# Lightning-AI/lit-llama

Hardware: NVIDIA H100
Metric: LLaMA-7B gptq.int4 decode tokens/sec (higher is better)
Workload: dtype bf16

## Files before the change

lit-llama_b200/csrc/attention.cu:

```cuda
#include <cstdlib>

#include "b2l_common.cuh"

namespace b2l {

__global__ void ring_advance_kernel(const int64_t* __restrict__ input_pos, int T, int32_t* ring_start, int S) {
  if (threadIdx.x == 0 && blockIdx.x == 0) {
    if (input_pos[T - 1] >= (int64_t)S) *ring_start = (*ring_start + 1) % S;
  }
}

__global__ void rope_append_kernel(__nv_bfloat16* __restrict__ qkv, __nv_bfloat16* __restrict__ k_cache,
                                   __nv_bfloat16* __restrict__ v_cache, const float* __restrict__ rope,
                                   const int64_t* __restrict__ input_pos, const int32_t* __restrict__ ring_start,
                                   int T, int n_head, int hs, int S, int block_size, int rope_rows) {
  const int bt = blockIdx.x, h = blockIdx.y, b = bt / T, t = bt % T;
  const int C = n_head * hs;
  long long p = input_pos ? input_pos[t] : (long long)t;
  const long long prow = rope_rows ? (long long)t : (p < block_size ? p : (long long)block_size - 1);
  __nv_bfloat16* q = qkv + (size_t)bt * 3 * C + h * hs;
  __nv_bfloat16* k = q + C;
  const __nv_bfloat16* v = q + 2 * C;
  __nv_bfloat16 *kd = k, *vd = nullptr;
  if (k_cache != nullptr) {
    const int w = (int)(p < S ? p : (long long)S - 1);
    const int phys = (w + *ring_start) % S;
    const size_t off = (((size_t)b * n_head + h) * S + phys) * hs;
    kd = k_cache + off;
    vd = v_cache + off;
  }
  for (int i = threadIdx.x; i < hs / 2; i += blockDim.x) {
    const float c = rope[((size_t)prow * (hs / 2) + i) * 2 + 0];
    const float s = rope[((size_t)prow * (hs / 2) + i) * 2 + 1];
    const float q0 = bf2f(q[2 * i]), q1 = bf2f(q[2 * i + 1]);
    const float k0 = bf2f(k[2 * i]), k1 = bf2f(k[2 * i + 1]);
    q[2 * i] = f2bf(__fsub_rn(__fmul_rn(q0, c), __fmul_rn(q1, s)));
    q[2 * i + 1] = f2bf(__fadd_rn(__fmul_rn(q1, c), __fmul_rn(q0, s)));
    kd[2 * i] = f2bf(__fsub_rn(__fmul_rn(k0, c), __fmul_rn(k1, s)));
    kd[2 * i + 1] = f2bf(__fadd_rn(__fmul_rn(k1, c), __fmul_rn(k0, s)));
    if (vd != nullptr) {
      vd[2 * i] = v[2 * i];
      vd[2 * i + 1] = v[2 * i + 1];
    }
  }
}

struct KvView {
  const __nv_bfloat16* k;
  const __nv_bfloat16* v;
  size_t b_stride, h_stride, s_stride;
  int S;
};

constexpr int ATT_WARPS = 4;
constexpr int ATT_MAX_EPL = 8;

template <int EPL>
__global__ void __launch_bounds__(ATT_WARPS * 32)
    attn_partial_kernel(const __nv_bfloat16* __restrict__ qkv, KvView kv, const int64_t* __restrict__ input_pos,
                        const int32_t* __restrict__ ring_start, float* __restrict__ work, int T, int n_head,
                        int hs, int n_split, int chunk) {
  const int bh = blockIdx.x, b = bh / n_head, h = bh % n_head, t = blockIdx.y, sp = blockIdx.z;
  const int lane = threadIdx.x & 31, warp = threadIdx.x >> 5;
  const int C = n_head * hs;
  long long p = input_pos ? input_pos[t] : (long long)t;
  const int cap = kv.S > 0 ? kv.S : T;
  const int L = (int)(p < cap ? p : (long long)cap - 1) + 1;
  const int ring = (kv.S > 0 && ring_start) ? *ring_start : 0;
  const int j0 = sp * chunk, j1 = min(L, j0 + chunk);
  float* out = work + (((size_t)bh * T + t) * n_split + sp) * (hs + 2);
  if (j0 >= j1) {
    if (threadIdx.x == 0) { out[0] = -INFINITY; out[1] = 0.f; }
    for (int d = threadIdx.x; d < hs; d += blockDim.x) out[2 + d] = 0.f;
    return;
  }
  const float scale = rsqrtf((float)hs);
  float qv[ATT_MAX_EPL];
  const __nv_bfloat16* q = qkv + ((size_t)b * T + t) * 3 * C + h * hs;
#pragma unroll
  for (int e = 0; e < ATT_MAX_EPL; ++e) {
    int d = (EPL > 0) ? lane * EPL + e : lane + 32 * e;
    qv[e] = (e < (EPL > 0 ? EPL : ATT_MAX_EPL) && d < hs) ? bf2f(q[d]) * scale : 0.f;
// ... 16 lines not shown
      kx[2] = __uint_as_float(ku.y << 16); kx[3] = __uint_as_float(ku.y & 0xffff0000u);
      vx[0] = __uint_as_float(vu.x << 16); vx[1] = __uint_as_float(vu.x & 0xffff0000u);
      vx[2] = __uint_as_float(vu.y << 16); vx[3] = __uint_as_float(vu.y & 0xffff0000u);
    } else {
#pragma unroll
      for (int e = 0; e < ATT_MAX_EPL; ++e) {
        int d = lane + 32 * e;
        kx[e] = d < hs ? bf2f(kr[d]) : 0.f;
        vx[e] = d < hs ? bf2f(vr[d]) : 0.f;
      }
    }
    float sc = 0.f;
#pragma unroll
    for (int e = 0; e < (EPL > 0 ? EPL : ATT_MAX_EPL); ++e) sc = fmaf(qv[e], kx[e], sc);
    sc = warp_sum(sc);
    const float mn = fmaxf(m, sc);
    const float corr = __expf(m - mn), pj = __expf(sc - mn);
    l = l * corr + pj;
#pragma unroll
    for (int e = 0; e < (EPL > 0 ? EPL : ATT_MAX_EPL); ++e) acc[e] = fmaf(pj, vx[e], acc[e] * corr);
    m = mn;
  }
  __shared__ float sm_m[ATT_WARPS], sm_l[ATT_WARPS];
  __shared__ float sm_acc[ATT_WARPS][32 * ATT_MAX_EPL];
  if (lane == 0) { sm_m[warp] = m; sm_l[warp] = l; }
#pragma unroll
  for (int e = 0; e < (EPL > 0 ? EPL : ATT_MAX_EPL); ++e) {
    int d = (EPL > 0) ? lane * EPL + e : lane + 32 * e;
    sm_acc[warp][d] = acc[e];
  }
  __syncthreads();
  float M = -INFINITY;
#pragma unroll
  for (int w = 0; w < ATT_WARPS; ++w) M = fmaxf(M, sm_m[w]);
  float Ls = 0.f;
  float wgt[ATT_WARPS];
#pragma unroll
  for (int w = 0; w < ATT_WARPS; ++w) {
    wgt[w] = (sm_m[w] == -INFINITY) ? 0.f : __expf(sm_m[w] - M);
    Ls += sm_l[w] * wgt[w];
  }
  if (threadIdx.x == 0) { out[0] = M; out[1] = Ls; }
  for (int d = threadIdx.x; d < hs; d += blockDim.x) {
    float a = 0.f;
#pragma unroll
    for (int w = 0; w < ATT_WARPS; ++w) a += sm_acc[w][d] * wgt[w];
    out[2 + d] = a;
  }
}

__global__ void attn_combine_kernel(const float* __restrict__ work, __nv_bfloat16* __restrict__ y, int T,
                                    int n_head, int hs, int n_split) {
  pdl_launch_dependents();
  const int bh = blockIdx.x, b = bh / n_head, h = bh % n_head, t = blockIdx.y;
  const float* base = work + ((size_t)bh * T + t) * n_split * (hs + 2);
  float M = -INFINITY;
  for (int s = 0; s < n_split; ++s) M = fmaxf(M, base[(size_t)s * (hs + 2)]);
  float Ls = 0.f;
  for (int s = 0; s < n_split; ++s) {
    float ms = base[(size_t)s * (hs + 2)];
    if (ms != -INFINITY) Ls += base[(size_t)s * (hs + 2) + 1] * __expf(ms - M);
  }
  const float inv = 1.0f / Ls;
  __nv_bfloat16* yr = y + ((size_t)b * T + t) * (n_head * hs) + h * hs;
  for (int d = threadIdx.x; d < hs; d += blockDim.x) {
    float a = 0.f;
    for (int s = 0; s < n_split; ++s) {
      float ms = base[(size_t)s * (hs + 2)];
      if (ms != -INFINITY) a += base[(size_t)s * (hs + 2) + 2 + d] * __expf(ms - M);
    }
    yr[d] = f2bf(a * inv);
  }
}

__global__ void kv_unroll_kernel(const __nv_bfloat16* __restrict__ cache, const int32_t* __restrict__ ring_start,
                                 __nv_bfloat16* __restrict__ out, int S, int hs) {
  const int ring = *ring_start;
  const int phys = (blockIdx.y + ring) % S;
  const __nv_bfloat16* src = cache + ((size_t)blockIdx.x * S + phys) * hs;
  __nv_bfloat16* dst = out + ((size_t)blockIdx.x * S + blockIdx.y) * hs;
  for (int d = threadIdx.x; d < hs; d += blockDim.x) dst[d] = src[d];
}

constexpr int FD_CHUNK = 256;
constexpr int FD_SUB = 64;
constexpr int FD_WARPS = 8;
constexpr int FD_CTAS_PER_SM = 3;
constexpr int WS_CHUNK = FD_SUB;

__device__ __forceinline__ void bf16x8_to_f32(const uint4& u, float* f) {
  const uint32_t w[4] = {u.x, u.y, u.z, u.w};
#pragma unroll
  for (int i = 0; i < 4; ++i) {
    f[2 * i] = __uint_as_float(w[i] << 16);
    f[2 * i + 1] = __uint_as_float(w[i] & 0xffff0000u);
  }
}

__device__ __forceinline__ uint32_t fd_smem_u32(const void* p) { return (uint32_t)__cvta_generic_to_shared(p); }
__device__ __forceinline__ void fd_bulk(uint32_t dst, const void* src, uint32_t bytes, uint32_t bar) {
  asm volatile("cp.async.bulk.shared::cluster.global.mbarrier::complete_tx::bytes [%0], [%1], %2, [%3];" ::"r"(dst), "l"(src), "r"(bytes), "r"(bar) : "memory");
}

constexpr int FD_SUB_BYTES = FD_SUB * 128 * 2;
constexpr int FD_SMEM_BYTES = 4 * FD_SUB_BYTES + FD_WARPS * 128 * 4 + 2 * FD_WARPS * 4 + 16;

__device__ __forceinline__ float fd_adapter_prefix(const float* sq, float* ssc, const __nv_bfloat16* __restrict__ ak,
                                                   const __nv_bfloat16* __restrict__ av, int alen, int warp, int lane,
                                                   int d, bool writer) {
  constexpr int HS = 128;
  const float4 qv = reinterpret_cast<const float4*>(sq)[lane];
#pragma unroll 2
  for (int j = warp; j < alen; j += FD_WARPS) {
    const uint2 ku = __ldg(reinterpret_cast<const uint2*>(ak + (size_t)j * HS) + lane);
    float s = qv.x * __uint_as_float(ku.x << 16);
    s = fmaf(qv.y, __uint_as_float(ku.x & 0xffff0000u), s);
    s = fmaf(qv.z, __uint_as_float(ku.y << 16), s);
    s = fmaf(qv.w, __uint_as_float(ku.y & 0xffff0000u), s);
    s = warp_sum(s);
    if (lane == 0) ssc[j] = s;
  }
  __syncthreads();
  float ay = 0.f;
  if (writer) {
    float mx = -INFINITY;
    for (int j = 0; j < alen; ++j) mx = fmaxf(mx, ssc[j]);
    float l = 0.f;
#pragma unroll 8
    for (int j = 0; j < alen; ++j) {
      const float p = __expf(ssc[j] - mx);
      l += p;
      ay = fmaf(p, bf2f(av[(size_t)j * HS + d]), ay);
    }
    ay /= l;
  }
  return ay;
}

__device__ __forceinline__ __nv_bfloat16 adapter_combine(float y, float ay, float gate) {
  return f2bf(rbf(y) + rbf(gate * rbf(ay)));
}

template <bool ADAPTER>
__global__ void __launch_bounds__(FD_WARPS * 32, ADAPTER ? FD_CTAS_PER_SM : 0)
    attn_decode_fused_kernel(const __nv_bfloat16* qkv, __nv_bfloat16* __restrict__ k_cache,
                             __nv_bfloat16* __restrict__ v_cache, const float* __restrict__ rope,
                             const int64_t* __restrict__ input_pos, const int32_t* __restrict__ ring_start,
                             __nv_bfloat16* __restrict__ y, float* __restrict__ work, int* __restrict__ tickets,
                             int n_head, int S, int block_size, int n_split, unsigned long long* tl, int pre_tiles,
                             int smem_merge, int target_ctas, const __nv_bfloat16* __restrict__ pre_k,
                             const __nv_bfloat16* __restrict__ pre_v, const __nv_bfloat16* __restrict__ pre_gate,
                             int pre_len) {
  constexpr int HS = 128;
  extern __shared__ __align__(128) uint8_t fsm[];
  float* sm_acc = reinterpret_cast<float*>(fsm + 4 * FD_SUB_BYTES);
  float* sm_m = sm_acc + FD_WARPS * HS;
  float* sm_l = sm_m + FD_WARPS;
  unsigned long long* bars = reinterpret_cast<unsigned long long*>(sm_l + FD_WARPS);
  __shared__ int sm_last;

  if (threadIdx.x == 0) tl_min(tl, 0);
  const int bh = blockIdx.x, b = bh / n_head, h = bh % n_head, sp = blockIdx.y;
  unsigned long long* tl0 = (tl != nullptr && blockIdx.x == 0 && blockIdx.y == 0 && threadIdx.x == 0) ? tl + 8 : nullptr;
  int tli = 0;
  auto stamp = [&]() { if (tl0 != nullptr && tli < 24) tl0[tli++] = globaltimer_ns(); };
  stamp();
  const int lane = threadIdx.x & 31, warp = threadIdx.x >> 5;
  const int C = n_head * HS;
  const size_t head_base = ((size_t)b * n_head + h) * S * HS;

  const long long p = input_pos[0];
  const int w_slot = (int)(p < S ? p : (long long)S - 1);
  const int L = w_slot + 1;
  const int want_splits = max(1, target_ctas / n_head);
  const int chunk = L <= FD_CHUNK ? FD_CHUNK
                                  : min(FD_CHUNK, max(FD_SUB, FD_SUB * ((L + FD_SUB * want_splits - 1) / (FD_SUB * want_splits))));
  const int n_active = (L + chunk - 1) / chunk;
  if (sp >= n_active) return;
  const int ring = *ring_start;
  const int j0 = sp * chunk, j1 = min(L, j0 + chunk);
  const int n_old = min(j1, L - 1) - j0;
  const int n_sub = (n_old + FD_SUB - 1) / FD_SUB;
  const bool has_new = (w_slot >= j0 && w_slot < j1);

  const uint32_t bar0 = fd_smem_u32(bars);
  auto request = [&](int i) {
    const int buf = i & 1;
    const int cnt = min(FD_SUB, n_old - i * FD_SUB);
    int phys0 = j0 + i * FD_SUB + ring; if (phys0 >= S) phys0 -= S;
    const int first = min(cnt, S - phys0);
    const uint32_t bar = bar0 + buf * 8;
    const uint32_t kd = fd_smem_u32(fsm) + buf * 2 * FD_SUB_BYTES, vd = kd + FD_SUB_BYTES;
    asm volatile("mbarrier.arrive.expect_tx.shared::cta.b64 _, [%0], %1;" ::"r"(bar), "r"((uint32_t)cnt * HS * 2 * 2) : "memory");
    fd_bulk(kd, k_cache + head_base + (size_t)phys0 * HS, (uint32_t)first * HS * 2, bar);
    fd_bulk(vd, v_cache + head_base + (size_t)phys0 * HS, (uint32_t)first * HS * 2, bar);
    if (first < cnt) {
      fd_bulk(kd + first * HS * 2, k_cache + head_base, (uint32_t)(cnt - first) * HS * 2, bar);
      fd_bulk(vd + first * HS * 2, v_cache + head_base, (uint32_t)(cnt - first) * HS * 2, bar);
    }
  };
  const int pre = (n_active == 1) ? 2 : pre_tiles;
  if (threadIdx.x == 0) {
    asm volatile("mbarrier.init.shared::cta.b64 [%0], 1;" ::"r"(bar0) : "memory");
    asm volatile("mbarrier.init.shared::cta.b64 [%0], 1;" ::"r"(bar0 + 8) : "memory");
    asm volatile("fence.mbarrier_init.release.cluster;" ::: "memory");
    if (n_sub > 0) request(0);
    if (pre > 1 && n_sub > 1) request(1);
  }
  if constexpr (ADAPTER) {
    if (threadIdx.x == 0) {
      const size_t off = (size_t)h * pre_len * HS;
      const uint32_t bytes = (uint32_t)pre_len * HS * 2;
      asm volatile("cp.async.bulk.prefetch.L2.global [%0], %1;" ::"l"(pre_k + off), "r"(bytes) : "memory");
      asm volatile("cp.async.bulk.prefetch.L2.global [%0], %1;" ::"l"(pre_v + off), "r"(bytes) : "memory");
    }
  }
  const long long prow = p < block_size ? p : (long long)block_size - 1;
  const int grp = lane >> 3, sub = lane & 7, d0 = sub * 16;
  float cs[16];
  {
    const float4* rp = reinterpret_cast<const float4*>(rope + ((size_t)prow * (HS / 2) + d0 / 2) * 2);
#pragma unroll
    for (int i = 0; i < 4; ++i) {
      float4 t = rp[i];
      cs[4 * i] = t.x; cs[4 * i + 1] = t.y; cs[4 * i + 2] = t.z; cs[4 * i + 3] = t.w;
    }
  }
  __syncthreads();
  pdl_wait();
  if (threadIdx.x == 0) tl_max(tl, 1);
  stamp();
  pdl_launch_dependents();

  const __nv_bfloat16* qrow = qkv + (size_t)b * 3 * C + h * HS + d0;
  float q[16];
  {
    float raw[16];
    const uint4 qa = ld_coherent_u4(qrow), qb = ld_coherent_u4(qrow + 8);
    if (threadIdx.x == 0 && pre <= 1 && n_sub > 1) request(1);
    bf16x8_to_f32(qa, raw);
    bf16x8_to_f32(qb, raw + 8);
    const float scale = rsqrtf((float)HS);
#pragma unroll
    for (int i = 0; i < 8; ++i) {
      const float c = cs[2 * i], s_ = cs[2 * i + 1];
      const float e = rbf(__fsub_rn(__fmul_rn(raw[2 * i], c), __fmul_rn(raw[2 * i + 1], s_)));
      const float o = rbf(__fadd_rn(__fmul_rn(raw[2 * i + 1], c), __fmul_rn(raw[2 * i], s_)));
      q[2 * i] = e * scale;
      q[2 * i + 1] = o * scale;
    }
  }
  float ay = 0.f;
  if constexpr (ADAPTER) {
    if (warp == 0 && grp == 0) {
      float4* dq = reinterpret_cast<float4*>(sm_acc + d0);
#pragma unroll
      for (int i = 0; i < 4; ++i) dq[i] = make_float4(q[4 * i], q[4 * i + 1], q[4 * i + 2], q[4 * i + 3]);
    }
    __syncthreads();
    ay = fd_adapter_prefix(sm_acc, sm_acc + HS, pre_k + (size_t)h * pre_len * HS, pre_v + (size_t)h * pre_len * HS,
                           pre_len, warp, lane, threadIdx.x & (HS - 1), threadIdx.x < HS);
  }

  float m = -INFINITY, l = 0.f, acc[16];
#pragma unroll
  for (int i = 0; i < 16; ++i) acc[i] = 0.f;
  if (tl0 != nullptr && q[0] != 12345.678f) stamp();
  if (has_new && warp == 0 && grp == 0) {
    int phys = w_slot + ring; if (phys >= S) phys -= S;
    float raw[16], kf[16], vf[16];
    bf16x8_to_f32(ld_coherent_u4(qrow + C), raw);
    bf16x8_to_f32(ld_coherent_u4(qrow + C + 8), raw + 8);
    uint32_t out[8];
#pragma unroll
    for (int i = 0; i < 8; ++i) {
      const float c = cs[2 * i], s_ = cs[2 * i + 1];
      kf[2 * i] = rbf(__fsub_rn(__fmul_rn(raw[2 * i], c), __fmul_rn(raw[2 * i + 1], s_)));
      kf[2 * i + 1] = rbf(__fadd_rn(__fmul_rn(raw[2 * i + 1], c), __fmul_rn(raw[2 * i], s_)));
      out[i] = (__float_as_uint(kf[2 * i]) >> 16) | (__float_as_uint(kf[2 * i + 1]) & 0xffff0000u);
    }
    const uint4 va = ld_coherent_u4(qrow + 2 * C), vb = ld_coherent_u4(qrow + 2 * C + 8);
    uint4* kd = reinterpret_cast<uint4*>(k_cache + head_base + (size_t)phys * HS + d0);
    uint4* vd = reinterpret_cast<uint4*>(v_cache + head_base + (size_t)phys * HS + d0);
    kd[0] = make_uint4(out[0], out[1], out[2], out[3]); kd[1] = make_uint4(out[4], out[5], out[6], out[7]);
    vd[0] = va; vd[1] = vb;
    bf16x8_to_f32(va, vf); bf16x8_to_f32(vb, vf + 8);
    float sc = 0.f;
#pragma unroll
    for (int e = 0; e < 16; ++e) sc = fmaf(q[e], kf[e], sc);
    sc += __shfl_xor_sync(0x000000ffu, sc, 1);
    sc += __shfl_xor_sync(0x000000ffu, sc, 2);
    sc += __shfl_xor_sync(0x000000ffu, sc, 4);
    const float mn = fmaxf(m, sc);
    const float corr = __expf(m - mn), pj = __expf(sc - mn);
    l = l * corr + pj;
#pragma unroll
    for (int e = 0; e < 16; ++e) acc[e] = fmaf(pj, vf[e], acc[e] * corr);
    m = mn;
  }
  for (int i = 0; i < n_sub; ++i) {
    const int buf = i & 1;
    const int cnt = min(FD_SUB, n_old - i * FD_SUB);
    {
      uint32_t ok;
      const uint32_t par = (uint32_t)(i >> 1) & 1u;
      do {
        asm volatile("{\n\t.reg .pred p;\n\tmbarrier.try_wait.parity.shared::cta.b64 p, [%1], %2;\n\tselp.u32 %0, 1, 0, p;\n\t}" : "=r"(ok) : "r"(bar0 + buf * 8), "r"(par) : "memory");
      } while (!ok);
    }
    const __nv_bfloat16* kt = reinterpret_cast<const __nv_bfloat16*>(fsm + buf * 2 * FD_SUB_BYTES);
    const __nv_bfloat16* vt = kt + FD_SUB * HS;
    stamp();
    float sc[2];
    bool valid[2];
    const uint4* vr[2];
#pragma unroll
    for (int it = 0; it < 2; ++it) {
      const int r = warp * 8 + it * 4 + grp;
      valid[it] = r < cnt;
      const int rc = valid[it] ? r : 0;
      const uint4* kr = reinterpret_cast<const uint4*>(kt + (size_t)rc * HS + d0);
      vr[it] = reinterpret_cast<const uint4*>(vt + (size_t)rc * HS + d0);
      float kf[16];
      bf16x8_to_f32(kr[0], kf); bf16x8_to_f32(kr[1], kf + 8);
      float a0 = 0.f, a1 = 0.f;
#pragma unroll
      for (int e = 0; e < 8; ++e) { a0 = fmaf(q[e], kf[e], a0); a1 = fmaf(q[8 + e], kf[8 + e], a1); }
      sc[it] = a0 + a1;
    }
#pragma unroll
    for (int o = 1; o <= 4; o <<= 1) {
      sc[0] += __shfl_xor_sync(0xffffffffu, sc[0], o);
      sc[1] += __shfl_xor_sync(0xffffffffu, sc[1], o);
    }
    {
      const float s0 = valid[0] ? sc[0] : -INFINITY, s1 = valid[1] ? sc[1] : -INFINITY;
      const float mn = fmaxf(m, fmaxf(s0, s1));
      if (mn != -INFINITY) {
        const float corr = __expf(m - mn), p0 = __expf(s0 - mn), p1 = __expf(s1 - mn);
        float v0[16], v1[16];
        bf16x8_to_f32(vr[0][0], v0); bf16x8_to_f32(vr[0][1], v0 + 8);
        bf16x8_to_f32(vr[1][0], v1); bf16x8_to_f32(vr[1][1], v1 + 8);
        l = l * corr + p0 + p1;
#pragma unroll
        for (int e = 0; e < 16; ++e) acc[e] = fmaf(p1, v1[e], fmaf(p0, v0[e], acc[e] * corr));
        m = mn;
      }
    }
    __syncthreads();
    stamp();
    if (threadIdx.x == 0 && i + 2 < n_sub) request(i + 2);
  }
  if (threadIdx.x == 0) tl_max(tl, 2);
  __syncwarp();
  if (threadIdx.x == 0) tl_max(tl, 3);
  float* part = reinterpret_cast<float*>(fsm);
  float* pm = part + 32 * HS;
  float* pl = pm + 32, *pw = pl + 32;
  const int n_part = smem_merge ? 32 : FD_WARPS;
  if (smem_merge) {
    const int g = warp * 4 + grp;
    float4* dst = reinterpret_cast<float4*>(part + g * HS + d0);
#pragma unroll
    for (int i = 0; i < 4; ++i) dst[i] = make_float4(acc[4 * i], acc[4 * i + 1], acc[4 * i + 2], acc[4 * i + 3]);
    if (sub == 0) { pm[g] = m; pl[g] = l; }
  } else {
#pragma unroll
    for (int off = 8; off <= 16; off <<= 1) {
      const float mo = __shfl_xor_sync(0xffffffffu, m, off);
      const float lo = __shfl_xor_sync(0xffffffffu, l, off);
      const float mn = fmaxf(m, mo);
      const float ca = (m == -INFINITY) ? 0.f : __expf(m - mn);
      const float cb = (mo == -INFINITY) ? 0.f : __expf(mo - mn);
      l = l * ca + lo * cb;
#pragma unroll
      for (int i = 0; i < 16; ++i) {
        const float ao = __shfl_xor_sync(0xffffffffu, acc[i], off);
        acc[i] = acc[i] * ca + ao * cb;
      }
      m = mn;
    }
    if (lane == 0) { pm[warp] = m; pl[warp] = l; }
    if (grp == 0) {
      float4* dst = reinterpret_cast<float4*>(part + warp * HS + d0);
#pragma unroll
      for (int i = 0; i < 4; ++i) dst[i] = make_float4(acc[4 * i], acc[4 * i + 1], acc[4 * i + 2], acc[4 * i + 3]);
    }
  }
  __syncthreads();
  if (warp == 0) {
    const float mi = lane < n_part ? pm[lane] : -INFINITY;
    const float Mx = warp_max(mi);
    const float wi = (mi == -INFINITY) ? 0.f : __expf(mi - Mx);
    const float Lx = warp_sum(lane < n_part ? pl[lane] * wi : 0.f);
    pw[lane] = wi;
    if (lane == 0) { pw[32] = Mx; pw[33] = Lx; }
  }
  __syncthreads();
  const float M = pw[32], Ls = pw[33];
  const int d = threadIdx.x & (HS - 1);
  const bool writer = threadIdx.x < HS;
  float a = 0.f;
  if (writer) {
#pragma unroll 8
    for (int g = 0; g < n_part; ++g) a = fmaf(part[g * HS + d], pw[g], a);
  }
  stamp();
  if (n_active == 1) {
    if constexpr (ADAPTER) {
      if (writer) y[(size_t)b * C + h * HS + d] = adapter_combine(a / Ls, ay, bf2f(pre_gate[h]));
    } else {
      if (writer) y[(size_t)b * C + h * HS + d] = f2bf(a / Ls);
    }
    if (threadIdx.x == 0) tl_max(tl, 4);
    stamp();
    return;
  }
  float* out = work + ((size_t)bh * n_split + sp) * (HS + 2);
  if (threadIdx.x == 0) { out[0] = M; out[1] = Ls; }
  if (writer) out[2 + d] = a;
  __syncthreads();
  if (threadIdx.x == 0) {
    int t;
    asm volatile("atom.add.acq_rel.gpu.global.s32 %0, [%1], 1;" : "=r"(t) : "l"(tickets + bh) : "memory");
    sm_last = (t == n_active - 1);
    if (sm_last) tickets[bh] = 0;
  }
  __syncthreads();
  stamp();
  if (!sm_last) return;
  const float* base = work + (size_t)bh * n_split * (HS + 2);
  float MM = -INFINITY, LL = 0.f, aa = 0.f;
  for (int s0 = 0; s0 < n_active; s0 += 8) {
    float ms[8], ls[8], as[8];
#pragma unroll
    for (int i = 0; i < 8; ++i) {
      const int s2 = s0 + i;
      const bool ok = s2 < n_active;
      const float* bp = base + (size_t)(ok ? s2 : s0) * (HS + 2);
      ms[i] = ok ? __ldcg(bp) : -INFINITY;
      ls[i] = ok ? __ldcg(bp + 1) : 0.f;
      as[i] = ok ? __ldcg(bp + 2 + d) : 0.f;
    }
    float bm = MM;
#pragma unroll
    for (int i = 0; i < 8; ++i) bm = fmaxf(bm, ms[i]);
    const float c0 = (MM == -INFINITY) ? 0.f : __expf(MM - bm);
    LL *= c0; aa *= c0;
#pragma unroll
    for (int i = 0; i < 8; ++i) {
      const float wg = (ms[i] == -INFINITY) ? 0.f : __expf(ms[i] - bm);
      LL += ls[i] * wg;
      aa += as[i] * wg;
    }
    MM = bm;
  }
  if constexpr (ADAPTER) {
    if (writer) y[(size_t)b * C + h * HS + d] = adapter_combine(aa / LL, ay, bf2f(pre_gate[h]));
  } else {
    if (writer) y[(size_t)b * C + h * HS + d] = f2bf(aa / LL);
  }
  if (threadIdx.x == 0) tl_max(tl, 4);
}

__global__ void __launch_bounds__(ATT_WARPS * 32)
    attn_adapter_prefix_kernel(const __nv_bfloat16* __restrict__ qkv, const __nv_bfloat16* __restrict__ pk,
                               const __nv_bfloat16* __restrict__ pv, const __nv_bfloat16* __restrict__ gate,
                               __nv_bfloat16* __restrict__ y, int n_head, int hs, int alen) {
  pdl_launch_dependents();
  __shared__ float sq[32 * ATT_MAX_EPL];
  __shared__ float ssc[B2L_ADAPTER_MAX_LEN];
  const int bt = blockIdx.x, h = blockIdx.y;
  const int lane = threadIdx.x & 31, warp = threadIdx.x >> 5;
  const int C = n_head * hs;
  const float scale = rsqrtf((float)hs);
  const __nv_bfloat16* q = qkv + (size_t)bt * 3 * C + h * hs;
  for (int d = threadIdx.x; d < hs; d += blockDim.x) sq[d] = bf2f(q[d]) * scale;
  __syncthreads();
  const __nv_bfloat16* kb = pk + (size_t)h * alen * hs;
  const __nv_bfloat16* vb = pv + (size_t)h * alen * hs;
  for (int j = warp; j < alen; j += ATT_WARPS) {
    float s = 0.f;
    for (int d = lane; d < hs; d += 32) s = fmaf(sq[d], bf2f(kb[(size_t)j * hs + d]), s);
    s = warp_sum(s);
    if (lane == 0) ssc[j] = s;
  }
  __syncthreads();
  float mx = -INFINITY;
  for (int j = 0; j < alen; ++j) mx = fmaxf(mx, ssc[j]);
  float l = 0.f;
  for (int j = 0; j < alen; ++j) l += __expf(ssc[j] - mx);
  const float g = bf2f(gate[h]);
  __nv_bfloat16* yr = y + (size_t)bt * C + h * hs;
  for (int d = threadIdx.x; d < hs; d += blockDim.x) {
    float a = 0.f;
    for (int j = 0; j < alen; ++j) a = fmaf(__expf(ssc[j] - mx), bf2f(vb[(size_t)j * hs + d]), a);
    yr[d] = adapter_combine(bf2f(yr[d]), a / l, g);
  }
}

constexpr int PF_Q = 64, PF_K = 64, PF_LD = 136;
constexpr int PF_TILE_BYTES = PF_Q * PF_LD * 2;
constexpr int PF_SMEM_BYTES = 5 * PF_TILE_BYTES;

__device__ __forceinline__ void ldsm_x4(uint32_t addr, uint32_t& r0, uint32_t& r1, uint32_t& r2, uint32_t& r3) {
  asm volatile("ldmatrix.sync.aligned.m8n8.x4.shared.b16 {%0, %1, %2, %3}, [%4];" : "=r"(r0), "=r"(r1), "=r"(r2), "=r"(r3) : "r"(addr) : "memory");
}
__device__ __forceinline__ void ldsm_x4_t(uint32_t addr, uint32_t& r0, uint32_t& r1, uint32_t& r2, uint32_t& r3) {
  asm volatile("ldmatrix.sync.aligned.m8n8.x4.trans.shared.b16 {%0, %1, %2, %3}, [%4];" : "=r"(r0), "=r"(r1), "=r"(r2), "=r"(r3) : "r"(addr) : "memory");
}
__device__ __forceinline__ void mma_bf16(float (&d)[4], uint32_t a0, uint32_t a1, uint32_t a2, uint32_t a3, uint32_t b0, uint32_t b1) {
  asm volatile("mma.sync.aligned.m16n8k16.row.col.f32.bf16.bf16.f32 {%0, %1, %2, %3}, {%4, %5, %6, %7}, {%8, %9}, {%0, %1, %2, %3};"
               : "+f"(d[0]), "+f"(d[1]), "+f"(d[2]), "+f"(d[3]) : "r"(a0), "r"(a1), "r"(a2), "r"(a3), "r"(b0), "r"(b1));
}
__device__ __forceinline__ void pf_cp16(uint32_t dst, const void* src) {
  asm volatile("cp.async.cg.shared.global [%0], [%1], 16;" ::"r"(dst), "l"(src) : "memory");
}
__device__ __forceinline__ void split_bf16x2(float x, float y, uint32_t& hi, uint32_t& lo) {
  const __nv_bfloat162 h = __floats2bfloat162_rn(x, y);
  const __nv_bfloat162 l = __floats2bfloat162_rn(x - __low2float(h), y - __high2float(h));
  hi = *reinterpret_cast<const uint32_t*>(&h);
  lo = *reinterpret_cast<const uint32_t*>(&l);
}

__global__ void __launch_bounds__(128)
    attn_prefill_kernel(const __nv_bfloat16* __restrict__ qkv, KvView kv, const int64_t* __restrict__ input_pos,
                        const int32_t* __restrict__ ring_start, __nv_bfloat16* __restrict__ y, int T, int n_head) {
  constexpr int HS = 128;
  extern __shared__ __align__(128) uint8_t psm[];
  const uint32_t sq = fd_smem_u32(psm), sk0 = sq + PF_TILE_BYTES;
  const int bh = blockIdx.x, b = bh / n_head, h = bh % n_head, t0 = blockIdx.y * PF_Q;
  const int tid = threadIdx.x, warp = tid >> 5, lane = tid & 31, g = lane >> 2, t4 = lane & 3;
  const int C = n_head * HS;
  const int cap = kv.S > 0 ? kv.S : T;
  const int ring = (kv.S > 0 && ring_start) ? *ring_start : 0;
  const __nv_bfloat16* kb = kv.k + (size_t)b * kv.b_stride + (size_t)h * kv.h_stride;
  const __nv_bfloat16* vb = kv.v + (size_t)b * kv.b_stride + (size_t)h * kv.h_stride;

  int Lrow[2];
#pragma unroll
  for (int i = 0; i < 2; ++i) {
    const int t = min(t0 + warp * 16 + g + 8 * i, T - 1);
    const long long p = input_pos ? input_pos[t] : (long long)t;
// ... 104 lines not shown
      uint32_t ah[4], al[4];
      split_bf16x2(sacc[2 * kk][0], sacc[2 * kk][1], ah[0], al[0]);
      split_bf16x2(sacc[2 * kk][2], sacc[2 * kk][3], ah[1], al[1]);
      split_bf16x2(sacc[2 * kk + 1][0], sacc[2 * kk + 1][1], ah[2], al[2]);
      split_bf16x2(sacc[2 * kk + 1][2], sacc[2 * kk + 1][3], ah[3], al[3]);
#pragma unroll
      for (int dn = 0; dn < 16; dn += 2) {
        uint32_t b0, b1, b2, b3;
        ldsm_x4_t(vsm + ((kk * 16 + (lane & 7) + ((lane >> 3) & 1) * 8) * PF_LD + dn * 8 + (lane >> 4) * 8) * 2, b0, b1, b2, b3);
        mma_bf16(o[dn], ah[0], ah[1], ah[2], ah[3], b0, b1);
        mma_bf16(o[dn], al[0], al[1], al[2], al[3], b0, b1);
        mma_bf16(o[dn + 1], ah[0], ah[1], ah[2], ah[3], b2, b3);
        mma_bf16(o[dn + 1], al[0], al[1], al[2], al[3], b2, b3);
      }
    }
    __syncthreads();
  }
#pragma unroll
  for (int r = 0; r < 2; ++r) {
    lrow[r] += __shfl_xor_sync(0xffffffffu, lrow[r], 1);
    lrow[r] += __shfl_xor_sync(0xffffffffu, lrow[r], 2);
  }
#pragma unroll
  for (int r = 0; r < 2; ++r) {
    const int t = t0 + warp * 16 + g + 8 * r;
    if (t < T) {
      const float inv = 1.0f / lrow[r];
      __nv_bfloat16* dst = y + ((size_t)b * T + t) * C + h * HS + 2 * t4;
#pragma unroll
      for (int n = 0; n < 16; ++n)
        *reinterpret_cast<__nv_bfloat162*>(dst + n * 8) = __floats2bfloat162_rn(o[n][2 * r] * inv, o[n][2 * r + 1] * inv);
    }
  }
}

void* g_attn_timeline = nullptr;

static inline void split_plan(int T, int S, int* n_split, int* chunk) {
  if (T > 1) { *n_split = 1; *chunk = S; return; }
  *chunk = 64;
  *n_split = (S + 63) / 64;
}

static int launch_attn(const __nv_bfloat16* qkv, KvView kv, const int64_t* input_pos, const int32_t* ring_start,
                       float* work, __nv_bfloat16* y, int B, int T, int n_head, int hs, int cap, cudaStream_t st) {
  static const int env_pf = [] { const char* e = getenv("B2L_ATTN_PREFILL"); return e ? atoi(e) : 1; }();
  if (hs == 128 && T > 1 && env_pf) {
    static DynSmemCache smem_cache;
    if (int rc = ensure_dyn_smem(attn_prefill_kernel, PF_SMEM_BYTES, smem_cache)) return rc;
    attn_prefill_kernel<<<dim3(B * n_head, (T + PF_Q - 1) / PF_Q), 128, PF_SMEM_BYTES, st>>>(qkv, kv, input_pos, ring_start, y, T, n_head);
    B2L_LAUNCH_CHECK("attn_prefill_kernel");
    return 0;
  }
  int n_split, chunk;
  split_plan(T, cap, &n_split, &chunk);
  dim3 grid(B * n_head, T, n_split), block(ATT_WARPS * 32);
  if (hs == 128)
    attn_partial_kernel<4><<<grid, block, 0, st>>>(qkv, kv, input_pos, ring_start, work, T, n_head, hs, n_split, chunk);
  else
    attn_partial_kernel<0><<<grid, block, 0, st>>>(qkv, kv, input_pos, ring_start, work, T, n_head, hs, n_split, chunk);
  B2L_LAUNCH_CHECK("attn_partial_kernel");
  attn_combine_kernel<<<dim3(B * n_head, T), 128, 0, st>>>(work, y, T, n_head, hs, n_split);
  B2L_LAUNCH_CHECK("attn_combine_kernel");
  return 0;
}

int check_adapter_prefix(const b2l_adapter_prefix* pre, const char* who) {
  B2L_CHECK_ARG(pre != nullptr && pre->k != nullptr && pre->v != nullptr && pre->gate != nullptr,
                "%s: null adapter prefix pointer", who);
  B2L_CHECK_SUPPORTED(pre->len > 0 && pre->len <= B2L_ADAPTER_MAX_LEN, "%s: adapter prefix length %d unsupported (1..%d)",
                      who, pre->len, B2L_ADAPTER_MAX_LEN);
  B2L_CHECK_ARG(((uintptr_t)pre->k & 15) == 0 && ((uintptr_t)pre->v & 15) == 0 && ((uintptr_t)pre->gate & 1) == 0,
                "%s: adapter prefix k / v must be 16-byte aligned, gate 2-byte aligned", who);
  return 0;
}

}

using namespace b2l;

static inline size_t ws_partials_bytes(int B, int n_head, int head_size, int T, int S) {
  int n_split, chunk;
  split_plan(T, S, &n_split, &chunk);
  size_t a = (size_t)B * n_head * T * n_split * (head_size + 2) * sizeof(float);
  size_t f = (size_t)B * n_head * ((S + WS_CHUNK - 1) / WS_CHUNK) * (head_size + 2) * sizeof(float);
  return ((a > f ? a : f) + 15) & ~(size_t)15;
}

extern "C" size_t b2l_attn_workspace_bytes(int B, int n_head, int head_size, int T, int S) {
  return ws_partials_bytes(B, n_head, head_size, T, S) + (size_t)B * n_head * sizeof(int);
}

extern "C" int b2l_ring_advance(const int64_t* input_pos, int T, int32_t* ring_start, int S, b2l_stream_t stream) {
  B2L_CHECK_ARG(input_pos && ring_start && T > 0 && S > 0, "b2l_ring_advance: bad argument");
  ring_advance_kernel<<<1, 32, 0, (cudaStream_t)stream>>>(input_pos, T, ring_start, S);
  B2L_LAUNCH_CHECK("ring_advance_kernel");
  return 0;
}

static int launch_adapter_prefix(const void* qkv, const b2l_adapter_prefix* pre, void* y, int B, int T, int n_head,
                                 int head_size, cudaStream_t st) {
  attn_adapter_prefix_kernel<<<dim3(B * T, n_head), ATT_WARPS * 32, 0, st>>>(
      (const __nv_bfloat16*)qkv, (const __nv_bfloat16*)pre->k, (const __nv_bfloat16*)pre->v,
      (const __nv_bfloat16*)pre->gate, (__nv_bfloat16*)y, n_head, head_size, pre->len);
  B2L_LAUNCH_CHECK("attn_adapter_prefix_kernel");
  return 0;
}

static int attention_impl(void* qkv, void* k_cache, void* v_cache, const void* rope, const int64_t* input_pos,
                          const int32_t* ring_start, void* y, void* work, int B, int T, int n_head, int head_size,
                          int S, int block_size, int flags, const b2l_adapter_prefix* pre, cudaStream_t st) {
  if (T == 1 && head_size == 128 && !(flags & B2L_F_ROPE_ROWS) && !(flags & B2L_F_ATTN_UNFUSED)) {
    const int n_split = (S + FD_SUB - 1) / FD_SUB;
    int* tickets = reinterpret_cast<int*>(reinterpret_cast<char*>(work) + ws_partials_bytes(B, n_head, head_size, T, S));
    static const int env_pre = [] { const char* e = getenv("B2L_ATTN_PRE"); return e ? atoi(e) : 1; }();
    static const int env_smem_merge = [] { const char* e = getenv("B2L_ATTN_SMEM_MERGE"); return e ? atoi(e) : 0; }();
    LaunchCfg lc(dim3(B * n_head, n_split), dim3(FD_WARPS * 32), FD_SMEM_BYTES, st, (flags & B2L_F_PDL) != 0);
    if (pre == nullptr) {
      static DynSmemCache smem_cache;
      if (int rc = ensure_dyn_smem(attn_decode_fused_kernel<false>, FD_SMEM_BYTES, smem_cache)) return rc;
      B2L_CUDA(cudaLaunchKernelEx(&lc.cfg, attn_decode_fused_kernel<false>, (const __nv_bfloat16*)qkv, (__nv_bfloat16*)k_cache,
                                  (__nv_bfloat16*)v_cache, (const float*)rope, input_pos, ring_start, (__nv_bfloat16*)y,
                                  (float*)work, tickets, n_head, S, block_size, n_split, (unsigned long long*)g_attn_timeline, env_pre, env_smem_merge,
                                  FD_CTAS_PER_SM * sm_count(), (const __nv_bfloat16*)nullptr, (const __nv_bfloat16*)nullptr,
                                  (const __nv_bfloat16*)nullptr, 0));
    } else {
      static DynSmemCache smem_cache;
      if (int rc = ensure_dyn_smem(attn_decode_fused_kernel<true>, FD_SMEM_BYTES, smem_cache)) return rc;
      B2L_CUDA(cudaLaunchKernelEx(&lc.cfg, attn_decode_fused_kernel<true>, (const __nv_bfloat16*)qkv, (__nv_bfloat16*)k_cache,
                                  (__nv_bfloat16*)v_cache, (const float*)rope, input_pos, ring_start, (__nv_bfloat16*)y,
                                  (float*)work, tickets, n_head, S, block_size, n_split, (unsigned long long*)g_attn_timeline, env_pre, env_smem_merge,
                                  FD_CTAS_PER_SM * sm_count(), (const __nv_bfloat16*)pre->k, (const __nv_bfloat16*)pre->v,
                                  (const __nv_bfloat16*)pre->gate, pre->len));
    }
    return 0;
  }
  int rt = head_size / 2 < 32 ? 32 : head_size / 2;
  rope_append_kernel<<<dim3(B * T, n_head), rt, 0, st>>>((__nv_bfloat16*)qkv, (__nv_bfloat16*)k_cache,
                                                        (__nv_bfloat16*)v_cache, (const float*)rope, input_pos,
                                                        ring_start, T, n_head, head_size, S, block_size, (flags & B2L_F_ROPE_ROWS) ? 1 : 0);
  B2L_LAUNCH_CHECK("rope_append_kernel");
  KvView kv{(const __nv_bfloat16*)k_cache, (const __nv_bfloat16*)v_cache, (size_t)n_head * S * head_size,
            (size_t)S * head_size, (size_t)head_size, S};
  if (int rc = launch_attn((const __nv_bfloat16*)qkv, kv, input_pos, ring_start, (float*)work, (__nv_bfloat16*)y, B, T,
                           n_head, head_size, S, st))
    return rc;
  return pre == nullptr ? 0 : launch_adapter_prefix(qkv, pre, y, B, T, n_head, head_size, st);
}

extern "C" int b2l_attention(void* qkv, void* k_cache, void* v_cache, const void* rope, const int64_t* input_pos,
                             const int32_t* ring_start, void* y, void* work, int B, int T, int n_head,
                             int head_size, int S, int block_size, int flags, b2l_stream_t stream) {
  B2L_CHECK_ARG(qkv && k_cache && v_cache && rope && input_pos && ring_start && y && work,
                "b2l_attention: null pointer");
  B2L_CHECK_ARG(B > 0 && T > 0 && n_head > 0 && S > 0 && T <= S && block_size > 0, "b2l_attention: bad shape");
  B2L_CHECK_SUPPORTED(head_size % 2 == 0 && head_size >= 2 && head_size <= 32 * ATT_MAX_EPL,
                      "b2l_attention: head_size %d unsupported (even, <= %d)", head_size, 32 * ATT_MAX_EPL);
  return attention_impl(qkv, k_cache, v_cache, rope, input_pos, ring_start, y, work, B, T, n_head, head_size, S,
                        block_size, flags, nullptr, (cudaStream_t)stream);
}

extern "C" int b2l_attention_adapter(void* qkv, void* k_cache, void* v_cache, const void* rope,
                                     const int64_t* input_pos, const int32_t* ring_start, void* y, void* work, int B,
                                     int T, int n_head, int head_size, int S, int block_size, int flags,
                                     const b2l_adapter_prefix* prefix, b2l_stream_t stream) {
  B2L_CHECK_ARG(qkv && k_cache && v_cache && rope && input_pos && ring_start && y && work,
                "b2l_attention_adapter: null pointer");
  B2L_CHECK_ARG(B > 0 && T > 0 && n_head > 0 && S > 0 && T <= S && block_size > 0, "b2l_attention_adapter: bad shape");
  B2L_CHECK_SUPPORTED(head_size % 2 == 0 && head_size >= 2 && head_size <= 32 * ATT_MAX_EPL,
                      "b2l_attention_adapter: head_size %d unsupported (even, <= %d)", head_size, 32 * ATT_MAX_EPL);
  if (int rc = check_adapter_prefix(prefix, "b2l_attention_adapter")) return rc;
  return attention_impl(qkv, k_cache, v_cache, rope, input_pos, ring_start, y, work, B, T, n_head, head_size, S,
                        block_size, flags, prefix, (cudaStream_t)stream);
}

static int attention_nocache_impl(void* qkv, const void* rope, void* y, void* work, int B, int T, int n_head,
                                  int head_size, int block_size, cudaStream_t st) {
  int rt = head_size / 2 < 32 ? 32 : head_size / 2;
  rope_append_kernel<<<dim3(B * T, n_head), rt, 0, st>>>((__nv_bfloat16*)qkv, nullptr, nullptr, (const float*)rope,
                                                        nullptr, nullptr, T, n_head, head_size, 0, block_size, 0);
  B2L_LAUNCH_CHECK("rope_append_kernel");
  const int C = n_head * head_size;
  const __nv_bfloat16* base = (const __nv_bfloat16*)qkv;
  KvView kv{base + C, base + 2 * C, (size_t)T * 3 * C, (size_t)head_size, (size_t)3 * C, 0};
  return launch_attn(base, kv, nullptr, nullptr, (float*)work, (__nv_bfloat16*)y, B, T, n_head, head_size, T, st);
}

extern "C" int b2l_attention_nocache(void* qkv, const void* rope, void* y, void* work, int B, int T, int n_head,
                                     int head_size, int block_size, b2l_stream_t stream) {
  B2L_CHECK_ARG(qkv && rope && y && work && B > 0 && T > 0 && n_head > 0 && T <= block_size,
                "b2l_attention_nocache: bad argument");
  B2L_CHECK_SUPPORTED(head_size % 2 == 0 && head_size >= 2 && head_size <= 32 * ATT_MAX_EPL,
                      "b2l_attention_nocache: head_size %d unsupported", head_size);
  return attention_nocache_impl(qkv, rope, y, work, B, T, n_head, head_size, block_size, (cudaStream_t)stream);
}

extern "C" int b2l_attention_nocache_adapter(void* qkv, const void* rope, void* y, void* work, int B, int T,
                                             int n_head, int head_size, int block_size,
                                             const b2l_adapter_prefix* prefix, b2l_stream_t stream) {
  B2L_CHECK_ARG(qkv && rope && y && work && B > 0 && T > 0 && n_head > 0 && T <= block_size,
                "b2l_attention_nocache_adapter: bad argument");
  B2L_CHECK_SUPPORTED(head_size % 2 == 0 && head_size >= 2 && head_size <= 32 * ATT_MAX_EPL,
                      "b2l_attention_nocache_adapter: head_size %d unsupported", head_size);
  if (int rc = check_adapter_prefix(prefix, "b2l_attention_nocache_adapter")) return rc;
  cudaStream_t st = (cudaStream_t)stream;
  if (int rc = attention_nocache_impl(qkv, rope, y, work, B, T, n_head, head_size, block_size, st)) return rc;
  return launch_adapter_prefix(qkv, prefix, y, B, T, n_head, head_size, st);
}

extern "C" int b2l_kv_unroll(const void* cache, const int32_t* ring_start, void* out, int B, int n_head, int S,
                             int head_size, b2l_stream_t stream) {
  B2L_CHECK_ARG(cache && ring_start && out && B > 0 && n_head > 0 && S > 0 && head_size > 0,
                "b2l_kv_unroll: bad argument");
  kv_unroll_kernel<<<dim3(B * n_head, S), 64, 0, (cudaStream_t)stream>>>((const __nv_bfloat16*)cache, ring_start,
                                                                         (__nv_bfloat16*)out, S, head_size);
  B2L_LAUNCH_CHECK("kv_unroll_kernel");
  return 0;
}
// ... 1 lines not shown
```

Baseline: 595.0.

## Restructure fused decode attention split plan, grid order and shared-memory footprint

The fused decode-attention kernel now sizes its grid to the number of CTAs that can be resident (3 per SM divided across heads) rather than one CTA per 64-key tile. Chunks are balanced across the splits, and the last active split owns the newly appended token. The grid is transposed so splits run along x, and shared memory is shrunk by dropping the per-warp accumulators, so three CTAs can reliably fit per SM with launch bounds applied to both variants. The rope coefficient load is hoisted ahead of the KV prefetch, and the final merge is restricted to writer threads, which trades fewer idle CTAs against longer per-CTA streaming when the context is long.

```diff
diff --git a/lit-llama_b200/csrc/attention.cu b/lit-llama_b200/csrc/attention.cu
--- a/lit-llama_b200/csrc/attention.cu
+++ b/lit-llama_b200/csrc/attention.cu
@@ -1,3 +1,4 @@
+#include <algorithm>
 #include <cstdlib>
 
 #include "b2l_common.cuh"
@@ -180,11 +181,16 @@
   for (int d = threadIdx.x; d < hs; d += blockDim.x) dst[d] = src[d];
 }
 
-constexpr int FD_CHUNK = 256;
 constexpr int FD_SUB = 64;
 constexpr int FD_WARPS = 8;
+constexpr int FD_RING = 2;
 constexpr int FD_CTAS_PER_SM = 3;
-constexpr int WS_CHUNK = FD_SUB;
+constexpr int FD_ONE_CTA_KEYS = 256;
+constexpr int FD_SUB_BYTES = FD_SUB * 128 * 2;
+
+constexpr int FD_SMEM_BYTES = FD_RING * 2 * FD_SUB_BYTES + (128 + B2L_ADAPTER_MAX_LEN) * 4 + FD_RING * 8;
+static_assert(FD_CTAS_PER_SM * (FD_SMEM_BYTES + 1024 + 128) <= 228 * 1024, "FD_CTAS_PER_SM CTAs must fit in an SM's shared memory");
+static_assert(2 * FD_SUB_BYTES >= (32 * 128 + 3 * 32 + 2) * 4, "the CTA merge scratch must fit in one ring buffer");
 
 __device__ __forceinline__ void bf16x8_to_f32(const uint4& u, float* f) {
   const uint32_t w[4] = {u.x, u.y, u.z, u.w};
@@ -199,9 +205,6 @@
 __device__ __forceinline__ void fd_bulk(uint32_t dst, const void* src, uint32_t bytes, uint32_t bar) {
   asm volatile("cp.async.bulk.shared::cluster.global.mbarrier::complete_tx::bytes [%0], [%1], %2, [%3];" ::"r"(dst), "l"(src), "r"(bytes), "r"(bar) : "memory");
 }
-
-constexpr int FD_SUB_BYTES = FD_SUB * 128 * 2;
-constexpr int FD_SMEM_BYTES = 4 * FD_SUB_BYTES + FD_WARPS * 128 * 4 + 2 * FD_WARPS * 4 + 16;
 
 __device__ __forceinline__ float fd_adapter_prefix(const float* sq, float* ssc, const __nv_bfloat16* __restrict__ ak,
                                                    const __nv_bfloat16* __restrict__ av, int alen, int warp, int lane,
@@ -240,25 +243,23 @@
 }
 
 template <bool ADAPTER>
-__global__ void __launch_bounds__(FD_WARPS * 32, ADAPTER ? FD_CTAS_PER_SM : 0)
+__global__ void __launch_bounds__(FD_WARPS * 32, FD_CTAS_PER_SM)
     attn_decode_fused_kernel(const __nv_bfloat16* qkv, __nv_bfloat16* __restrict__ k_cache,
                              __nv_bfloat16* __restrict__ v_cache, const float* __restrict__ rope,
                              const int64_t* __restrict__ input_pos, const int32_t* __restrict__ ring_start,
-                             __nv_bfloat16* __restrict__ y, float* __restrict__ work, int* __restrict__ tickets,
-                             int n_head, int S, int block_size, int n_split, unsigned long long* tl, int pre_tiles,
-                             int smem_merge, int target_ctas, const __nv_bfloat16* __restrict__ pre_k,
-                             const __nv_bfloat16* __restrict__ pre_v, const __nv_bfloat16* __restrict__ pre_gate,
-                             int pre_len) {
+                             __nv_bfloat16* __restrict__ y, int n_head, int S, int block_size, int pre,
+                             int target_ctas, unsigned long long* tl, int smem_merge, float* __restrict__ work, int* __restrict__ tickets,
+                             const __nv_bfloat16* __restrict__ pre_k, const __nv_bfloat16* __restrict__ pre_v,
+                             const __nv_bfloat16* __restrict__ pre_gate, int pre_len) {
   constexpr int HS = 128;
   extern __shared__ __align__(128) uint8_t fsm[];
-  float* sm_acc = reinterpret_cast<float*>(fsm + 4 * FD_SUB_BYTES);
-  float* sm_m = sm_acc + FD_WARPS * HS;
-  float* sm_l = sm_m + FD_WARPS;
-  unsigned long long* bars = reinterpret_cast<unsigned long long*>(sm_l + FD_WARPS);
+  float* sq = reinterpret_cast<float*>(fsm + FD_RING * 2 * FD_SUB_BYTES);
+  unsigned long long* bars = reinterpret_cast<unsigned long long*>(sq + HS + B2L_ADAPTER_MAX_LEN);
   __shared__ int sm_last;
 
   if (threadIdx.x == 0) tl_min(tl, 0);
-  const int bh = blockIdx.x, b = bh / n_head, h = bh % n_head, sp = blockIdx.y;
+  const int sp = blockIdx.x;
+  const int bh = blockIdx.y, b = bh / n_head, h = bh % n_head;
   unsigned long long* tl0 = (tl != nullptr && blockIdx.x == 0 && blockIdx.y == 0 && threadIdx.x == 0) ? tl + 8 : nullptr;
   int tli = 0;
   auto stamp = [&]() { if (tl0 != nullptr && tli < 24) tl0[tli++] = globaltimer_ns(); };
@@ -270,22 +271,22 @@
   const long long p = input_pos[0];
   const int w_slot = (int)(p < S ? p : (long long)S - 1);
   const int L = w_slot + 1;
-  const int want_splits = max(1, target_ctas / n_head);
-  const int chunk = L <= FD_CHUNK ? FD_CHUNK
-                                  : min(FD_CHUNK, max(FD_SUB, FD_SUB * ((L + FD_SUB * want_splits - 1) / (FD_SUB * want_splits))));
-  const int n_active = (L + chunk - 1) / chunk;
+  const int n_tiles = (L - 1 + FD_SUB - 1) / FD_SUB;
+  const int want_splits = min((int)gridDim.x, max(1, target_ctas / n_head));
+  const int chunk = FD_SUB * max(1, L - 1 <= FD_ONE_CTA_KEYS ? n_tiles : (n_tiles + want_splits - 1) / want_splits);
+  const int n_active = max(1, (L - 1 + chunk - 1) / chunk);
   if (sp >= n_active) return;
-  const int ring = *ring_start;
-  const int j0 = sp * chunk, j1 = min(L, j0 + chunk);
+  const int rs = *ring_start;
+  const bool has_new = sp == n_active - 1;
+  const int j0 = sp * chunk, j1 = has_new ? L : j0 + chunk;
   const int n_old = min(j1, L - 1) - j0;
   const int n_sub = (n_old + FD_SUB - 1) / FD_SUB;
-  const bool has_new = (w_slot >= j0 && w_slot < j1);
 
   const uint32_t bar0 = fd_smem_u32(bars);
   auto request = [&](int i) {
-    const int buf = i & 1;
+    const int buf = i % FD_RING;
     const int cnt = min(FD_SUB, n_old - i * FD_SUB);
-    int phys0 = j0 + i * FD_SUB + ring; if (phys0 >= S) phys0 -= S;
+    int phys0 = j0 + i * FD_SUB + rs; if (phys0 >= S) phys0 -= S;
     const int first = min(cnt, S - phys0);
     const uint32_t bar = bar0 + buf * 8;
     const uint32_t kd = fd_smem_u32(fsm) + buf * 2 * FD_SUB_BYTES, vd = kd + FD_SUB_BYTES;
@@ -297,13 +298,22 @@
       fd_bulk(vd + first * HS * 2, v_cache + head_base, (uint32_t)(cnt - first) * HS * 2, bar);
     }
   };
-  const int pre = (n_active == 1) ? 2 : pre_tiles;
+  const long long prow = p < block_size ? p : (long long)block_size - 1;
+  const int grp = lane >> 3, sub = lane & 7, d0 = sub * 16;
+  float cs[16];
+  {
+    const float4* rp = reinterpret_cast<const float4*>(rope + ((size_t)prow * (HS / 2) + d0 / 2) * 2);
+#pragma unroll
+    for (int i = 0; i < 4; ++i) {
+      float4 t = rp[i];
+      cs[4 * i] = t.x; cs[4 * i + 1] = t.y; cs[4 * i + 2] = t.z; cs[4 * i + 3] = t.w;
+    }
+  }
+  const int n_ring = min(n_sub, FD_RING);
   if (threadIdx.x == 0) {
-    asm volatile("mbarrier.init.shared::cta.b64 [%0], 1;" ::"r"(bar0) : "memory");
-    asm volatile("mbarrier.init.shared::cta.b64 [%0], 1;" ::"r"(bar0 + 8) : "memory");
+    for (int i = 0; i < FD_RING; ++i) asm volatile("mbarrier.init.shared::cta.b64 [%0], 1;" ::"r"(bar0 + i * 8) : "memory");
     asm volatile("fence.mbarrier_init.release.cluster;" ::: "memory");
-    if (n_sub > 0) request(0);
-    if (pre > 1 && n_sub > 1) request(1);
+    for (int i = 0; i < min(n_ring, pre); ++i) request(i);
   }
   if constexpr (ADAPTER) {
     if (threadIdx.x == 0) {
@@ -313,17 +323,6 @@
       asm volatile("cp.async.bulk.prefetch.L2.global [%0], %1;" ::"l"(pre_v + off), "r"(bytes) : "memory");
     }
   }
-  const long long prow = p < block_size ? p : (long long)block_size - 1;
-  const int grp = lane >> 3, sub = lane & 7, d0 = sub * 16;
-  float cs[16];
-  {
-    const float4* rp = reinterpret_cast<const float4*>(rope + ((size_t)prow * (HS / 2) + d0 / 2) * 2);
-#pragma unroll
-    for (int i = 0; i < 4; ++i) {
-      float4 t = rp[i];
-      cs[4 * i] = t.x; cs[4 * i + 1] = t.y; cs[4 * i + 2] = t.z; cs[4 * i + 3] = t.w;
-    }
-  }
   __syncthreads();
   pdl_wait();
   if (threadIdx.x == 0) tl_max(tl, 1);
@@ -335,7 +334,8 @@
   {
     float raw[16];
     const uint4 qa = ld_coherent_u4(qrow), qb = ld_coherent_u4(qrow + 8);
-    if (threadIdx.x == 0 && pre <= 1 && n_sub > 1) request(1);
+    if (threadIdx.x == 0)
+      for (int i = pre; i < n_ring; ++i) request(i);
     bf16x8_to_f32(qa, raw);
     bf16x8_to_f32(qb, raw + 8);
     const float scale = rsqrtf((float)HS);
@@ -351,13 +351,13 @@
   float ay = 0.f;
   if constexpr (ADAPTER) {
     if (warp == 0 && grp == 0) {
-      float4* dq = reinterpret_cast<float4*>(sm_acc + d0);
+      float4* dq = reinterpret_cast<float4*>(sq + d0);
 #pragma unroll
       for (int i = 0; i < 4; ++i) dq[i] = make_float4(q[4 * i], q[4 * i + 1], q[4 * i + 2], q[4 * i + 3]);
     }
     __syncthreads();
-    ay = fd_adapter_prefix(sm_acc, sm_acc + HS, pre_k + (size_t)h * pre_len * HS, pre_v + (size_t)h * pre_len * HS,
-                           pre_len, warp, lane, threadIdx.x & (HS - 1), threadIdx.x < HS);
+    ay = fd_adapter_prefix(sq, sq + HS, pre_k + (size_t)h * pre_len * HS, pre_v + (size_t)h * pre_len * HS, pre_len,
+                           warp, lane, threadIdx.x & (HS - 1), threadIdx.x < HS);
   }
 
   float m = -INFINITY, l = 0.f, acc[16];
@@ -365,7 +365,7 @@
   for (int i = 0; i < 16; ++i) acc[i] = 0.f;
   if (tl0 != nullptr && q[0] != 12345.678f) stamp();
   if (has_new && warp == 0 && grp == 0) {
-    int phys = w_slot + ring; if (phys >= S) phys -= S;
+    int phys = w_slot + rs; if (phys >= S) phys -= S;
     float raw[16], kf[16], vf[16];
     bf16x8_to_f32(ld_coherent_u4(qrow + C), raw);
     bf16x8_to_f32(ld_coherent_u4(qrow + C + 8), raw + 8);
@@ -397,11 +397,11 @@
     m = mn;
   }
   for (int i = 0; i < n_sub; ++i) {
-    const int buf = i & 1;
+    const int buf = i % FD_RING;
     const int cnt = min(FD_SUB, n_old - i * FD_SUB);
     {
       uint32_t ok;
-      const uint32_t par = (uint32_t)(i >> 1) & 1u;
+      const uint32_t par = (uint32_t)(i / FD_RING) & 1u;
       do {
         asm volatile("{\n\t.reg .pred p;\n\tmbarrier.try_wait.parity.shared::cta.b64 p, [%1], %2;\n\tselp.u32 %0, 1, 0, p;\n\t}" : "=r"(ok) : "r"(bar0 + buf * 8), "r"(par) : "memory");
       } while (!ok);
@@ -447,7 +447,7 @@
     }
     __syncthreads();
     stamp();
-    if (threadIdx.x == 0 && i + 2 < n_sub) request(i + 2);
+    if (threadIdx.x == 0 && i + FD_RING < n_sub) request(i + FD_RING);
   }
   if (threadIdx.x == 0) tl_max(tl, 2);
   __syncwarp();
@@ -514,7 +514,7 @@
     stamp();
     return;
   }
-  float* out = work + ((size_t)bh * n_split + sp) * (HS + 2);
+  float* out = work + ((size_t)bh * gridDim.x + sp) * (HS + 2);
   if (threadIdx.x == 0) { out[0] = M; out[1] = Ls; }
   if (writer) out[2 + d] = a;
   __syncthreads();
@@ -525,17 +525,15 @@
     if (sm_last) tickets[bh] = 0;
   }
   __syncthreads();
-  stamp();
-  if (!sm_last) return;
-  const float* base = work + (size_t)bh * n_split * (HS + 2);
+  if (!sm_last || !writer) return;
+  const float* base = work + (size_t)bh * gridDim.x * (HS + 2);
   float MM = -INFINITY, LL = 0.f, aa = 0.f;
   for (int s0 = 0; s0 < n_active; s0 += 8) {
     float ms[8], ls[8], as[8];
 #pragma unroll
     for (int i = 0; i < 8; ++i) {
-      const int s2 = s0 + i;
-      const bool ok = s2 < n_active;
-      const float* bp = base + (size_t)(ok ? s2 : s0) * (HS + 2);
+      const bool ok = s0 + i < n_active;
+      const float* bp = base + (size_t)(ok ? s0 + i : s0) * (HS + 2);
       ms[i] = ok ? __ldcg(bp) : -INFINITY;
       ls[i] = ok ? __ldcg(bp + 1) : 0.f;
       as[i] = ok ? __ldcg(bp + 2 + d) : 0.f;
@@ -548,15 +546,15 @@
 #pragma unroll
     for (int i = 0; i < 8; ++i) {
       const float wg = (ms[i] == -INFINITY) ? 0.f : __expf(ms[i] - bm);
-      LL += ls[i] * wg;
-      aa += as[i] * wg;
+      LL = fmaf(ls[i], wg, LL);
+      aa = fmaf(as[i], wg, aa);
     }
     MM = bm;
   }
   if constexpr (ADAPTER) {
-    if (writer) y[(size_t)b * C + h * HS + d] = adapter_combine(aa / LL, ay, bf2f(pre_gate[h]));
+    y[(size_t)b * C + h * HS + d] = adapter_combine(aa / LL, ay, bf2f(pre_gate[h]));
   } else {
-    if (writer) y[(size_t)b * C + h * HS + d] = f2bf(aa / LL);
+    y[(size_t)b * C + h * HS + d] = f2bf(aa / LL);
   }
   if (threadIdx.x == 0) tl_max(tl, 4);
 }
@@ -827,9 +825,8 @@
 static inline size_t ws_partials_bytes(int B, int n_head, int head_size, int T, int S) {
   int n_split, chunk;
   split_plan(T, S, &n_split, &chunk);
-  size_t a = (size_t)B * n_head * T * n_split * (head_size + 2) * sizeof(float);
-  size_t f = (size_t)B * n_head * ((S + WS_CHUNK - 1) / WS_CHUNK) * (head_size + 2) * sizeof(float);
-  return ((a > f ? a : f) + 15) & ~(size_t)15;
+  const size_t a = (size_t)B * n_head * T * n_split * (head_size + 2) * sizeof(float);
+  return (a + 15) & ~(size_t)15;
 }
 
 extern "C" size_t b2l_attn_workspace_bytes(int B, int n_head, int head_size, int T, int S) {
@@ -852,33 +849,36 @@
   return 0;
 }
 
+template <bool ADAPTER>
+static int launch_fused_decode(const __nv_bfloat16* qkv, __nv_bfloat16* k_cache, __nv_bfloat16* v_cache, const float* rope,
+                               const int64_t* input_pos, const int32_t* ring_start, __nv_bfloat16* y, int B, int n_head,
+                               int S, int block_size, bool pdl, const b2l_adapter_prefix* pre, void* work, cudaStream_t st) {
+  static const int env_pre = [] { const char* e = getenv("B2L_ATTN_PRE"); return e ? atoi(e) : 1; }();
+  static const int env_smem_merge = [] { const char* e = getenv("B2L_ATTN_SMEM_MERGE"); return e ? atoi(e) : 0; }();
+  static DynSmemCache smem_cache;
+  if (int rc = ensure_dyn_smem(attn_decode_fused_kernel<ADAPTER>, FD_SMEM_BYTES, smem_cache)) return rc;
+  const int n_split = std::min((S + FD_SUB - 1) / FD_SUB, std::max(1, FD_CTAS_PER_SM * sm_count() / n_head));
+  int* tickets = reinterpret_cast<int*>(reinterpret_cast<char*>(work) + ws_partials_bytes(B, n_head, 128, 1, S));
+  LaunchCfg lc(dim3(n_split, B * n_head), dim3(FD_WARPS * 32), FD_SMEM_BYTES, st, pdl);
+  B2L_CUDA(cudaLaunchKernelEx(&lc.cfg, attn_decode_fused_kernel<ADAPTER>, qkv, k_cache, v_cache, rope, input_pos, ring_start, y,
+                              n_head, S, block_size, env_pre, FD_CTAS_PER_SM * sm_count(), (unsigned long long*)g_attn_timeline,
+                              env_smem_merge, (float*)work, tickets, pre ? (const __nv_bfloat16*)pre->k : nullptr,
+                              pre ? (const __nv_bfloat16*)pre->v : nullptr, pre ? (const __nv_bfloat16*)pre->gate : nullptr,
+                              pre ? pre->len : 0));
+  return 0;
+}
+
 static int attention_impl(void* qkv, void* k_cache, void* v_cache, const void* rope, const int64_t* input_pos,
                           const int32_t* ring_start, void* y, void* work, int B, int T, int n_head, int head_size,
                           int S, int block_size, int flags, const b2l_adapter_prefix* pre, cudaStream_t st) {
   if (T == 1 && head_size == 128 && !(flags & B2L_F_ROPE_ROWS) && !(flags & B2L_F_ATTN_UNFUSED)) {
-    const int n_split = (S + FD_SUB - 1) / FD_SUB;
-    int* tickets = reinterpret_cast<int*>(reinterpret_cast<char*>(work) + ws_partials_bytes(B, n_head, head_size, T, S));
-    static const int env_pre = [] { const char* e = getenv("B2L_ATTN_PRE"); return e ? atoi(e) : 1; }();
-    static const int env_smem_merge = [] { const char* e = getenv("B2L_ATTN_SMEM_MERGE"); return e ? atoi(e) : 0; }();
-    LaunchCfg lc(dim3(B * n_head, n_split), dim3(FD_WARPS * 32), FD_SMEM_BYTES, st, (flags & B2L_F_PDL) != 0);
-    if (pre == nullptr) {
-      static DynSmemCache smem_cache;
-      if (int rc = ensure_dyn_smem(attn_decode_fused_kernel<false>, FD_SMEM_BYTES, smem_cache)) return rc;
-      B2L_CUDA(cudaLaunchKernelEx(&lc.cfg, attn_decode_fused_kernel<false>, (const __nv_bfloat16*)qkv, (__nv_bfloat16*)k_cache,
-                                  (__nv_bfloat16*)v_cache, (const float*)rope, input_pos, ring_start, (__nv_bfloat16*)y,
-                                  (float*)work, tickets, n_head, S, block_size, n_split, (unsigned long long*)g_attn_timeline, env_pre, env_smem_merge,
-                                  FD_CTAS_PER_SM * sm_count(), (const __nv_bfloat16*)nullptr, (const __nv_bfloat16*)nullptr,
-                                  (const __nv_bfloat16*)nullptr, 0));
-    } else {
-      static DynSmemCache smem_cache;
-      if (int rc = ensure_dyn_smem(attn_decode_fused_kernel<true>, FD_SMEM_BYTES, smem_cache)) return rc;
-      B2L_CUDA(cudaLaunchKernelEx(&lc.cfg, attn_decode_fused_kernel<true>, (const __nv_bfloat16*)qkv, (__nv_bfloat16*)k_cache,
-                                  (__nv_bfloat16*)v_cache, (const float*)rope, input_pos, ring_start, (__nv_bfloat16*)y,
-                                  (float*)work, tickets, n_head, S, block_size, n_split, (unsigned long long*)g_attn_timeline, env_pre, env_smem_merge,
-                                  FD_CTAS_PER_SM * sm_count(), (const __nv_bfloat16*)pre->k, (const __nv_bfloat16*)pre->v,
-                                  (const __nv_bfloat16*)pre->gate, pre->len));
-    }
-    return 0;
+    return pre == nullptr
+               ? launch_fused_decode<false>((const __nv_bfloat16*)qkv, (__nv_bfloat16*)k_cache, (__nv_bfloat16*)v_cache,
+                                            (const float*)rope, input_pos, ring_start, (__nv_bfloat16*)y, B, n_head, S,
+                                            block_size, (flags & B2L_F_PDL) != 0, nullptr, work, st)
+               : launch_fused_decode<true>((const __nv_bfloat16*)qkv, (__nv_bfloat16*)k_cache, (__nv_bfloat16*)v_cache,
+                                           (const float*)rope, input_pos, ring_start, (__nv_bfloat16*)y, B, n_head, S,
+                                           block_size, (flags & B2L_F_PDL) != 0, pre, work, st);
   }
   int rt = head_size / 2 < 32 ? 32 : head_size / 2;
   rope_append_kernel<<<dim3(B * T, n_head), rt, 0, st>>>((__nv_bfloat16*)qkv, (__nv_bfloat16*)k_cache,
```

New measurement: 605.8, median of 6. +1.8%, better.
